# MpokiAbel/UPMEM--OpenFHE

Hardware: AMD Instinct MI355X
Metric: 64-bit coeffs/sec for NTT+Hadamard+INTT, N=2^16, 16 towers; % HBM roofline (higher is better)
Workload: dtype u64; 1 GPU; configs[2]: N=2^16, towers=16, batch=1024 per GPU, c = INTT(NTT(a) (.) b); log_n=16, towers=16, batch_per_gpu=1024, global_batch=1024, parallelism=batch-sharded x1 (no data-path collective)

## Files before the change

upmem--openfhe_amd/csrc/ntt_kernels.hpp:

```cpp
#pragma once
#include "arith.hpp"

namespace ofhe {

struct TowerConst {
    u64 q;
    u64 ninv;
    u64 ninv_pre;
    u64 mu;
    u64 nq;
    u64 nq4;
    u32 nshift;
    u32 spq_sh;
    u64 qinv;
    u32 one;
    u32 pad_;
};
#ifndef OFHE_QA_TCF
#define OFHE_QA_TCF 0
#endif
#ifndef OFHE_QA_TCI
#define OFHE_QA_TCI 0
#endif
#ifndef OFHE_QA_BLK
// ... 195 lines not shown
}
template <class M_>
__device__ __forceinline__ void dit_round16(u64 (&v)[16], const u64* dtw, u32 st, u32 r, const M_& M) {
    dit_stage16<0, 1>(v, dtw + 2 * ((u64)st + r), st, M);
    dit_stage16<1, 0>(v, dtw + 2 * ((u64)2 * st + r), st, M);
    dit_stage16<2, 1>(v, dtw + 2 * ((u64)4 * st + r), st, M);
    dit_stage16<3, 0>(v, dtw + 2 * ((u64)8 * st + r), st, M);
}

template <bool SPQ, bool QA>
__device__ __forceinline__ void dit_round3(u64 (&v)[16], const u64* dtw, const Mod<SPQ, QA>& M) {
#pragma unroll
    for (int g = 0; g < 16; g += 2) triv_bfly(v[g], v[g + 1], 2 * M.q);
#pragma unroll
    for (int g = 0; g < 16; g += 4) triv_bfly(v[g], v[g + 2], M.q4);
    {
        const Tw w = ldtw(dtw, 3);
#pragma unroll
        for (int g = 0; g < 16; g += 4) ct_bfly<0>(v[g + 1], v[g + 3], w, M);
    }
#pragma unroll
    for (int g = 0; g < 16; g += 8) triv_bfly(v[g], v[g + 4], M.q8);
#pragma unroll
    for (int j = 1; j < 4; j++) {
        const Tw w = ldtw(dtw, 4 + j);
#pragma unroll
        for (int g = 0; g < 16; g += 8) ct_bfly<0>(v[g + j], v[g + j + 4], w, M);
    }
    {
        const u64 a = red16(v[0], M), b = red16(v[8], M);
        v[0] = a;
        v[8] = b;
        triv_bfly(v[0], v[8], M.q8);
    }
#pragma unroll
    for (int j = 1; j < 8; j++) ct_bfly<1>(v[j], v[j + 8], ldtw(dtw, 8 + j), M);
}

template <bool SPQ, bool QA>
__device__ __forceinline__ u64 twist_out(u64 x, Tw f, const Mod<SPQ, QA>& M) {
    return canon4m(shoup_lazy(x, f.w, f.wp, M), M);
}

template <int S, class M_, int CS = S & 1>
__device__ __forceinline__ void fwd_stage16(u64 (&v)[16], const u64* tw, u32 M0, const M_& M) {
    constexpr int half = 8 >> S;
    const u64* base = tw + 2 * ((u64)M0 << S);
#pragma unroll
    for (int j = 0; j < (1 << S); j++) {
        Tw w = ldtw(base, j);
#pragma unroll
        for (int k = j * 2 * half; k < j * 2 * half + half; k++) ct_bfly<CS>(v[k], v[k + half], w, M);
    }
}

template <int S, class M_>
__device__ __forceinline__ void inv_stage16(u64 (&v)[16], const u64* itw, u32 M0, const M_& M) {
    constexpr int half = 8 >> S;
    const u64* base = itw + 2 * ((u64)M0 << S);
#pragma unroll
    for (int j = 0; j < (1 << S); j++) {
        Tw w = ldtw(base, j);
#pragma unroll
        for (int k = j * 2 * half; k < j * 2 * half + half; k++) gs_bfly(v[k], v[k + half], w, M);
    }
}

#ifndef OFHE_LAZY_GS
#define OFHE_LAZY_GS 1
#endif
template <class M_>
__device__ __forceinline__ void gs_bfly_b(u64& x, u64& y, Tw w, const M_& M, bool in8) {
    const u64 s = x + y;
    const u64 d = x + (in8 ? M.q8 : M.q4) - y;
    x = in8 ? red16_gs(s, M) : s;
    y = shoup_lazy(d, w.w, w.wp, M);
}
template <int S, class M_>
__device__ __forceinline__ void inv_stage16_b(u64 (&v)[16], bool (&b8)[16], const u64* itw, u32 M0, const M_& M) {
    constexpr int half = 8 >> S;
    const u64* base = itw + 2 * ((u64)M0 << S);
#pragma unroll
    for (int j = 0; j < (1 << S); j++) {
        Tw w = ldtw(base, j);
#pragma unroll
        for (int k = j * 2 * half; k < j * 2 * half + half; k++) {
            gs_bfly_b(v[k], v[k + half], w, M, b8[k] || b8[k + half]);
            b8[k] = true;
            b8[k + half] = false;
        }
    }
}
template <class M_>
__device__ __forceinline__ void inv_round16_b(u64 (&v)[16], bool (&b8)[16], const u64* itw, u32 M0, const M_& M) {
    inv_stage16_b<3>(v, b8, itw, M0, M);
    inv_stage16_b<2>(v, b8, itw, M0, M);
    inv_stage16_b<1>(v, b8, itw, M0, M);
    inv_stage16_b<0>(v, b8, itw, M0, M);
}

template <class M_>
__device__ __forceinline__ void fwd_round16(u64 (&v)[16], const u64* tw, u32 M0, const M_& M) {
    fwd_stage16<0>(v, tw, M0, M);
    fwd_stage16<1>(v, tw, M0, M);
    fwd_stage16<2>(v, tw, M0, M);
    fwd_stage16<3>(v, tw, M0, M);
}
#ifndef OFHE_FWD_CANON
#define OFHE_FWD_CANON 1
#endif
template <class M_>
__device__ __forceinline__ void fwd_round16_canon(u64 (&v)[16], const u64* tw, u32 M0, const M_& M) {
    fwd_stage16<0>(v, tw, M0, M);
    fwd_stage16<1, M_, OFHE_FWD_CANON ? 0 : 1>(v, tw, M0, M);
    fwd_stage16<2>(v, tw, M0, M);
    fwd_stage16<3>(v, tw, M0, M);
}
template <class M_>
__device__ __forceinline__ void inv_round16(u64 (&v)[16], const u64* itw, u32 M0, const M_& M) {
    inv_stage16<3>(v, itw, M0, M);
    inv_stage16<2>(v, itw, M0, M);
    inv_stage16<1>(v, itw, M0, M);
    inv_stage16<0>(v, itw, M0, M);
}

#ifndef OFHE_TW3
#define OFHE_TW3 1
#endif
#ifndef OFHE_MONT
#define OFHE_MONT 1
#endif
#ifndef OFHE_COAL
#define OFHE_COAL 1
#endif
#ifndef OFHE_COAL_B
#define OFHE_COAL_B 1
#endif
constexpr bool kMontFused = OFHE_MONT && OFHE_COAL_B;
static_assert(!(kMontFused && OFHE_THR), "Montgomery Hadamard needs the forward output < 12q");
template <int S, class M_>
__device__ __forceinline__ void fwd_stage16_t3(u64 (&v)[16], const u64* tw3, u32 U, u32 u, const M_& M) {
    constexpr int half = 8 >> S;
    const u64* base = tw3 + 2 * (u64)(((1u << S) - 1) * U);
#pragma unroll
    for (int j = 0; j < (1 << S); j++) {
        Tw w = ldtw(base + 2 * (u64)j * U, u);
#pragma unroll
        for (int k = j * 2 * half; k < j * 2 * half + half; k++) ct_bfly<S & 1>(v[k], v[k + half], w, M);
    }
}
__device__ __forceinline__ u32 lds_pad(u32 p) { return p + (p >> 4); }
constexpr u32 LDS_WORDS = 4096 + 4096 / 16;

__device__ __forceinline__ void wave_stage_in(const u64* wsrc, u64* lds, u32 tid, u64 (&out)[16]) {
    const u32 lane = tid & 63, base = (tid >> 6) * 1024;
#pragma unroll
    for (int k = 0; k < 8; k++) {
        const u64x2 v = ld2_s(wsrc + 128 * k + 2 * lane);
        const u32 p = base + 128 * k + 2 * lane;
        lds[lds_pad(p)] = v.x;
        lds[lds_pad(p) + 1] = v.y;
    }
    __builtin_amdgcn_wave_barrier();
#pragma unroll
    for (int k = 0; k < 16; k++) out[k] = lds[tid * 17 + k];
    __builtin_amdgcn_wave_barrier();
}
template <int NPRE>
__device__ __forceinline__ void wave_stage_in_pre(const u64* wsrc, u64* lds, u32 tid, const u64x2 (&pre)[NPRE > 0 ? NPRE : 1],
                                                  u64 (&out)[16]) {
    const u32 lane = tid & 63, base = (tid >> 6) * 1024;
#pragma unroll
    for (int k = 0; k < 8; k++) {
        const u64x2 v = k < NPRE ? pre[k < NPRE ? k : 0] : ld2_s(wsrc + 128 * k + 2 * lane);
        const u32 p = base + 128 * k + 2 * lane;
        lds[lds_pad(p)] = v.x;
        lds[lds_pad(p) + 1] = v.y;
    }
    __builtin_amdgcn_wave_barrier();
#pragma unroll
    for (int k = 0; k < 16; k++) out[k] = lds[tid * 17 + k];
    __builtin_amdgcn_wave_barrier();
}
__device__ __forceinline__ void wave_stage_out(const u64 (&v)[16], u64* lds, u32 tid, u64* wdst) {
    const u32 lane = tid & 63, base = (tid >> 6) * 1024;
#pragma unroll
    for (int k = 0; k < 16; k++) lds[tid * 17 + k] = v[k];
    __builtin_amdgcn_wave_barrier();
#pragma unroll
    for (int k = 0; k < 8; k++) {
        const u32 p = base + 128 * k + 2 * lane;
        u64x2 w;
        w.x = lds[lds_pad(p)];
        w.y = lds[lds_pad(p) + 1];
        st2_s(wdst + 128 * k + 2 * lane, w);
    }
}

#ifndef OFHE_B_PF
#define OFHE_B_PF 8
#endif
#ifndef OFHE_KB_WAVES
#define OFHE_KB_WAVES 4
#endif
template <int MODE, bool SPQ, int NR, int SK = 0>
__device__ __forceinline__ void block_body(const PlanArgs& P, const u64* src, u64* dst, const u64* __restrict__ bdat,
                                           u32 batch, u32 wid, u64* lds, u32 tid) {
    static_assert(NR == 2 || NR == 3, "k_block covers the last 8 (NR=2) or 12 (NR=3) stages");
    static_assert(SK == 0 || (SK == 3 && NR == 3), "k_block: SK = 3 needs NR = 3");
    const u32 logn = P.log_n;
    const u32 N = 1u << logn;
    const u32 G = N >> 12;
    const u32 g = wid % G;
    const u32 pb = wid / G;
    const u32 t = pb / batch, b = pb % batch;
    const u64 inner = (u64)t * N + ((u64)g << 12);
    const u64 off = (u64)b * P.dstride + inner;
    const u64 boff = (u64)b * P.bstride + inner;
    const u64* blk = src + (u64)b * P.sstride + inner;
    u64* oblk = dst + off;
    const TowerConst tc = P.tc[t];
    const u64 q = tc.q;
    const auto M = load_mod<SPQ, (bool)OFHE_QA_BLK>(tc);
    const u64* tw = P.tw + (u64)t * N * 2;
    const u32 h = tid >> 4, r = tid & 15;
    const u32 L1 = tid + h;
    const u32 L2 = h * 272 + r;
    const u32 L3 = tid * 17;
    u64 v[16];

    if (MODE == MODE_FWD || MODE == MODE_FUSED || MODE == MODE_FWD_SUB) {
        if (NR == 3) {
#pragma unroll
            for (int k = 0; k < 16; k++) v[k] = ld_s(blk + tid + 256 * k);
            if (SK == 3)
                fwd_stage16<3>(v, tw, (N >> 12) + g, M);
            else
                fwd_round16(v, tw, (N >> 12) + g, M);
#pragma unroll
            for (int k = 0; k < 16; k++) lds[L1 + 272 * k] = v[k];
            __syncthreads();
#pragma unroll
            for (int k = 0; k < 16; k++) v[k] = lds[L2 + 17 * k];
        } else {
#pragma unroll
            for (int k = 0; k < 16; k++) v[k] = ld_s(blk + h * 256 + r + 16 * k);
        }
        fwd_round16(v, tw, (N >> 8) + g * 16 + h, M);
#pragma unroll
        for (int k = 0; k < 16; k++) lds[L2 + 17 * k] = v[k];
        __syncthreads();
#pragma unroll
        for (int k = 0; k < 16; k++) v[k] = lds[L3 + k];
        constexpr int BPF = ((MODE == MODE_FUSED && OFHE_COAL_B) || MODE == MODE_FWD_SUB) ? OFHE_B_PF : 0;
        u64x2 bpre[BPF > 0 ? BPF : 1];
#pragma unroll
        for (int k = 0; k < BPF; k++) bpre[k] = ld2_s(bdat + boff + (tid >> 6) * 1024 + 128 * k + 2 * (tid & 63));
        if (OFHE_TW3) {
            const u64* tw3 = P.tw3 + (u64)t * (N / 16) * 30;
            const u32 U = N >> 4, u = g * 256 + tid;
            fwd_stage16_t3<0>(v, tw3, U, u, M);
            fwd_stage16_t3<1>(v, tw3, U, u, M);
            fwd_stage16_t3<2>(v, tw3, U, u, M);
            fwd_stage16_t3<3>(v, tw3, U, u, M);
        } else {
            fwd_round16(v, tw, (N >> 4) + g * 256 + tid, M);
        }
        if (!(MODE == MODE_FUSED && kMontFused) && MODE != MODE_FWD_SUB) {
#pragma unroll
            for (int k = 0; k < 16; k++) v[k] = canon_fwd<SPQ>(v[k], M);
        }
        if (MODE == MODE_FWD_SUB) {
            static_assert(!OFHE_THR, "the lazy forward-subtract needs the forward output < 12q (OFHE_THR widens it)");
            u64 xx[16];
            wave_stage_in_pre<BPF>(bdat + boff + (tid >> 6) * 1024, lds, tid, bpre, xx);
            const u64 sc = P.scal[3 * t + 1], scp = P.scal[3 * t + 2];
            const u64 q12 = M.q8 + M.q4;
#pragma unroll
            for (int k = 0; k < 16; k++) v[k] = canon4m(shoup_lazy(xx[k] + q12 - v[k], sc, scp, M), M);
            wave_stage_out(v, lds, tid, oblk + (tid >> 6) * 1024);
            return;
        }
        if (MODE == MODE_FWD) {
            if (OFHE_COAL) {
                wave_stage_out(v, lds, tid, oblk + (tid >> 6) * 1024);
            } else {
                ulonglong2* o = reinterpret_cast<ulonglong2*>(oblk + tid * 16);
#pragma unroll
                for (int k = 0; k < 8; k++) o[k] = make_ulonglong2(v[2 * k], v[2 * k + 1]);
            }
            return;
        }
        if (OFHE_COAL_B) {
            u64 bb[16];
            wave_stage_in_pre<BPF>(bdat + boff + (tid >> 6) * 1024, lds, tid, bpre, bb);
            if (kMontFused) {
#pragma unroll
                for (int k = 0; k < 16; k++) v[k] = mont_mul(v[k], bb[k], q, tc.qinv);
            } else {
#pragma unroll
                for (int k = 0; k < 16; k++) v[k] = barrett_ref(v[k], bb[k], q, tc.mu, tc.nshift);
            }
        } else {
            const ulonglong2* bp = reinterpret_cast<const ulonglong2*>(bdat + boff + tid * 16);
#pragma unroll
            for (int k = 0; k < 8; k++) {
#ifdef OFHE_ABL_NOB
                ulonglong2 bb = make_ulonglong2(v[k] ^ off, v[k + 8] ^ tid);
#else
                ulonglong2 bb = bp[k];
#endif
                v[2 * k] = barrett_ref(v[2 * k], bb.x, q, tc.mu, tc.nshift);
                v[2 * k + 1] = barrett_ref(v[2 * k + 1], bb.y, q, tc.mu, tc.nshift);
            }
        }
    } else {
        if (OFHE_COAL) {
            wave_stage_in(blk + (tid >> 6) * 1024, lds, tid, v);
        } else {
            const ulonglong2* ip = reinterpret_cast<const ulonglong2*>(blk + tid * 16);
#pragma unroll
            for (int k = 0; k < 8; k++) {
                ulonglong2 a = ip[k];
                v[2 * k] = a.x;
                v[2 * k + 1] = a.y;
            }
        }
    }
    const u64* dtw = P.dtw + (u64)t * N * 2;
    dit_round3(v, dtw, M);
#pragma unroll
    for (int k = 0; k < 16; k++) lds[L3 + k] = v[k];
    __syncthreads();
#pragma unroll
    for (int k = 0; k < 16; k++) v[k] = lds[L2 + 17 * k];
    dit_round16(v, dtw, 16, r, M);
    const u64* tw_ = P.twist + (u64)t * N * 2 + 2 * ((u64)g << 12);
    if (NR == 2) {
#pragma unroll
        for (int k = 0; k < 16; k++) {
            const u32 p = h * 256 + r + 16 * k;
            const Tw f = ldtw(tw_, p);
            st_s(oblk + p, shoup_lazy(v[k], f.w, f.wp, M));
        }
        return;
    }
#pragma unroll
    for (int k = 0; k < 16; k++) lds[L2 + 17 * k] = v[k];
    __syncthreads();
#pragma unroll
    for (int k = 0; k < 16; k++) v[k] = lds[L1 + 272 * k];
    if (SK == 3)
        dit_stage16<0, 1>(v, dtw + 2 * ((u64)256 + tid), 256, M);
    else
        dit_round16(v, dtw, 256, tid, M);
#pragma unroll
    for (int k = 0; k < 16; k++) {
        const Tw f = ldtw(tw_, tid + 256 * k);
        v[k] = logn == 12 ? twist_out(v[k], f, M) : shoup_lazy(v[k], f.w, f.wp, M);
    }
#pragma unroll
    for (int k = 0; k < 16; k++) st_s(oblk + tid + 256 * k, v[k]);
}
template <int MODE, bool SPQ, int NR, int SK = 0>
__global__ __launch_bounds__(256, OFHE_KB_WAVES) void k_block(PlanArgs P, const u64* src, u64* dst,
                                                              const u64* __restrict__ bdat, u32 batch, u32 nwg) {
    OFHE_VGPR_FLOOR();
    __shared__ u64 lds[LDS_WORDS];
    block_body<MODE, SPQ, NR, SK>(P, src, dst, bdat, batch, xcd_remap(blockIdx.x, nwg), lds, threadIdx.x);
}

struct SwSrc {
    const u64* last;
    u64 lstride;
    u64 ql;
    const u64* tab;
    u64 pre, pre_p;
};
#ifndef OFHE_TCOLS_W
#define OFHE_TCOLS_W 16
#endif
constexpr u32 TCOLS_W = OFHE_TCOLS_W;
#ifndef OFHE_TCOLS_PADF
#define OFHE_TCOLS_PADF 1
#endif
static_assert(TCOLS_W == 16 || TCOLS_W == 32, "column tile width");
constexpr u32 TCOLS_LDS_WORDS = 16 * 16 * TCOLS_W + 16 * 16;
#ifndef OFHE_TCOLS_HALF
#define OFHE_TCOLS_HALF 0
#endif
#ifndef OFHE_TCOLS_HALF_WAVES
#define OFHE_TCOLS_HALF_WAVES 5
#endif
constexpr u32 TCOLS_LDS_INV_WORDS = OFHE_TCOLS_HALF ? 8 * 16 * TCOLS_W : TCOLS_LDS_WORDS;
template <bool INV, bool SPQ, bool SWS = false, int LOGN = 16>
__device__ __forceinline__ void tcols_body(const PlanArgs& P, const u64* src, u64* dst, u32 batch, u32 wid,
                                           const SwSrc& SWA, u64* lds, u32 tid) {
    static_assert(LOGN == 16 || LOGN == 17, "k_tcols: N = 2^16 or 2^17");
    constexpr u32 N = 1u << LOGN, S = N / 256, W = TCOLS_W;
    const u32 cb = wid % (S / W);
    const u32 pb = wid / (S / W);
    const u32 t = pb / batch, b = pb % batch;
    const u64 inner = (u64)t * N + cb * W;
    const u64* x = src + (u64)b * P.sstride + inner;
    u64* y = dst + (u64)b * P.dstride + inner;
    const TowerConst tc = P.tc[t];
    const auto M = load_mod<SPQ, INV ? (bool)OFHE_QA_TCI : (bool)OFHE_QA_TCF>(tc);
    const u32 h = tid / W, r = tid % W;
    const u32 L1 = tid, L2 = h * 16 * W + r;
    u64 v[16];
    if (!INV) {
        const u64* tw = P.tw + (u64)t * N * 2;
        constexpr u32 RP = OFHE_TCOLS_PADF ? 16 * W + 16 : 16 * W;
        if (SWS) {
            const u64 w = SWA.tab[6 * t + 1], wp = SWA.tab[6 * t + 2];
            const SwMod sm = sw_mod(SWA.ql, tc.q);
            const u64* lp = SWA.last + (u64)b * SWA.lstride + cb * W;
#pragma unroll
            for (int k = 0; k < 16; k++) {
                u64 e = lp[(u64)(h + 16 * k) * S + r];
                if (SWA.pre != 1) e = shoup_canon(e, SWA.pre, SWA.pre_p, SWA.ql);
                e = switch_mod1(e, sm);
                v[k] = w != 1 ? shoup_canon(e, w, wp, tc.q) : e;
            }
        } else {
#pragma unroll
            for (int k = 0; k < 16; k++) v[k] = ld_s(x + (u64)(h + 16 * k) * S + r);
        }
        fwd_round16_canon(v, tw, 1, M);
#pragma unroll
        for (int k = 0; k < 16; k++) lds[L1 + RP * k] = v[k];
        __syncthreads();
#pragma unroll
        for (int k = 0; k < 16; k++) v[k] = lds[h * RP + r + W * k];
        fwd_round16(v, tw, 16 + h, M);
#pragma unroll
        for (int k = 0; k < 16; k++) st_s(y + (u64)(16 * h + k) * S + r, v[k]);
    } else {
        const u64* itw = P.itw + (u64)t * N * 2;
#pragma unroll
        for (int k = 0; k < 16; k++) v[k] = ld_s(x + (u64)(16 * h + k) * S + r);
        if (OFHE_LAZY_GS) {
            bool b8[16];
#pragma unroll
            for (int k = 0; k < 16; k++) b8[k] = false;
            inv_round16_b(v, b8, itw, 16 + h, M);
            if (OFHE_TCOLS_HALF) {
                u64 o[16];
                if (h < 8) {
#pragma unroll
                    for (int k = 0; k < 16; k++) lds[L2 + W * k] = v[k];
                }
                __syncthreads();
#pragma unroll
                for (int k = 0; k < 8; k++) o[k] = lds[L1 + 16 * W * k];
                __syncthreads();
                if (h >= 8) {
#pragma unroll
                    for (int k = 0; k < 16; k++) lds[L2 - 8 * 16 * W + W * k] = v[k];
                }
                __syncthreads();
#pragma unroll
                for (int k = 8; k < 16; k++) o[k] = lds[L1 + 16 * W * (k - 8)];
#pragma unroll
                for (int k = 0; k < 16; k++) {
                    v[k] = o[k];
                    b8[k] = true;
                }
            } else {
#pragma unroll
                for (int k = 0; k < 16; k++) lds[L2 + W * k] = v[k];
                __syncthreads();
#pragma unroll
                for (int k = 0; k < 16; k++) {
                    v[k] = lds[L1 + 16 * W * k];
                    b8[k] = true;
                }
            }
            inv_round16_b(v, b8, itw, 1, M);
#pragma unroll
            for (int k = 0; k < 16; k++)
                st_s(y + (u64)(h + 16 * k) * S + r, b8[k] ? canon8m(v[k], M) : canon4m(v[k], M));
        } else {
            inv_round16(v, itw, 16 + h, M);
#pragma unroll
            for (int k = 0; k < 16; k++) lds[L2 + W * k] = v[k];
            __syncthreads();
#pragma unroll
            for (int k = 0; k < 16; k++) v[k] = lds[L1 + 16 * W * k];
            inv_round16(v, itw, 1, M);
#pragma unroll
            for (int k = 0; k < 16; k++) st_s(y + (u64)(h + 16 * k) * S + r, canon4m(v[k], M));
        }
    }
}

// ... 280 lines not shown
```

upmem--openfhe_amd/csrc/ofhe_hip.hip:

```cpp
#include <cstdio>
#include <cstdlib>
#include <cstring>
#include <new>
#include <thread>

#include "compose.hpp"
#include "bconv_cols.hpp"

using namespace ofhe;

#define OFHE_VERSION "ofhe-hip 0.2 gfx950"

namespace ofhe {
static thread_local std::string g_err;
int fail(int code, const std::string& msg) {
    g_err = msg;
    return code;
}
int post_launch() {
    hipError_t e = hipGetLastError();
    if (e != hipSuccess) return fail(OFHE_ERR_HIP, std::string("kernel launch: ") + hipGetErrorString(e));
    return OFHE_OK;
}
}
// ... 346 lines not shown
    } tables[] = {{(void**)&p->d_tc, tc.data(), sizeof(TowerConst) * towers},
                  {(void**)&p->d_tw, tw.data(), words(tw)},
                  {(void**)&p->d_itw, itw.data(), words(itw)},
                  {(void**)&p->d_tw3, tw3.data(), words(tw3)},
                  {(void**)&p->d_dtw, dtw.data(), words(dtw)},
                  {(void**)&p->d_twist, twist.data(), words(twist)},
                  {(void**)&p->d_twist_r, twist_r.data(), words(twist_r)}};
    int rc = OFHE_OK;
    for (const auto& t : tables)
        if (rc == OFHE_OK) rc = alloc_upload(t.dst, t.src, t.bytes, "plan upload", ctx->device);
    if (rc != OFHE_OK) {
        ofhe_hip_plan_destroy(p);
        return rc;
    }
    *plan = p;
    return OFHE_OK;
}

int ofhe_hip_plan_tune(ofhe_plan_t p, uint32_t chunk_batch, uint32_t streams) {
    if (!p || !p->ctx) return fail(OFHE_ERR_STATE, "plan is NULL or destroyed");
    if (streams < 1 || streams > 2) return fail(OFHE_ERR_ARG, "streams must be 1 or 2");
    HIPCHK(hipSetDevice(p->ctx->device));
    std::lock_guard<std::mutex> lk(p->fork_mu);
    if (streams == 2 && !p->st[0]) {
        hipStream_t st[2] = {nullptr, nullptr};
        hipEvent_t fork = nullptr, join[2] = {nullptr, nullptr};
        hipError_t e = hipSuccess;
        for (int i = 0; i < 2 && e == hipSuccess; i++) {
            e = hipStreamCreateWithFlags(&st[i], hipStreamNonBlocking);
            if (e == hipSuccess) e = hipEventCreateWithFlags(&join[i], hipEventDisableTiming);
        }
        if (e == hipSuccess) e = hipEventCreateWithFlags(&fork, hipEventDisableTiming);
        if (e != hipSuccess) {
            for (int i = 0; i < 2; i++) {
                if (st[i]) (void)hipStreamDestroy(st[i]);
                if (join[i]) (void)hipEventDestroy(join[i]);
            }
            if (fork) (void)hipEventDestroy(fork);
            return fail(OFHE_ERR_HIP, std::string("plan_tune: ") + hipGetErrorString(e));
        }
        for (int i = 0; i < 2; i++) {
            p->st[i] = st[i];
            p->ev_join[i] = join[i];
        }
        p->ev_fork = fork;
    }
    p->chunk_batch = chunk_batch;
    p->nstreams = streams;
    return OFHE_OK;
}

int ofhe_hip_plan_destroy(ofhe_plan_t p) {
    if (!p) return fail(OFHE_ERR_ARG, "plan is NULL");
    if (p->ctx) (void)hipSetDevice(p->ctx->device);
    for (int i = 0; i < 2; i++) {
        if (p->st[i]) (void)hipStreamSynchronize(p->st[i]);
        if (p->st[i]) (void)hipStreamDestroy(p->st[i]);
        if (p->ev_join[i]) (void)hipEventDestroy(p->ev_join[i]);
    }
    if (p->ev_fork) (void)hipEventDestroy(p->ev_fork);
    (void)hipFree(p->d_tc);
    (void)hipFree(p->d_tw);
    (void)hipFree(p->d_itw);
    (void)hipFree(p->d_tw3);
    (void)hipFree(p->d_dtw);
    (void)hipFree(p->d_twist);
    (void)hipFree(p->d_twist_r);
    for (auto& kv : p->tabs) (void)hipFree(kv.second);
    delete p;
    return OFHE_OK;
}

int ofhe_hip_plan_tables(ofhe_plan_t p, uint64_t* tab, uint64_t* tab_pre, uint64_t* itab,
                         uint64_t* itab_pre, uint64_t* ninv) {
    if (!p) return fail(OFHE_ERR_ARG, "plan is NULL");
    const size_t n = p->tab.size() * sizeof(u64);
    if (tab) memcpy(tab, p->tab.data(), n);
    if (tab_pre) memcpy(tab_pre, p->tab_pre.data(), n);
    if (itab) memcpy(itab, p->itab.data(), n);
    if (itab_pre) memcpy(itab_pre, p->itab_pre.data(), n);
    if (ninv) memcpy(ninv, p->ninv.data(), p->ninv.size() * sizeof(u64));
    return OFHE_OK;
}

static PlanArgs args_of(ofhe_plan_t p, u32 t0 = 0, u32 count = 0) {
    if (!count) count = p->towers - t0;
    const u64 N = 1ull << p->log_n;
    PlanArgs a;
    a.tc = p->d_tc + t0;
    a.tw = p->d_tw + 2 * N * t0;
    a.itw = p->d_itw + 2 * N * t0;
    a.tw3 = p->d_tw3 + (N >= 4096 ? (N / 16) * 30 * t0 : 0);
    a.sstride = a.dstride = a.bstride = N * count;
    a.scal = nullptr;
    a.dtw = p->d_dtw + 2 * N * t0;
    a.twist = p->d_twist + 2 * N * t0;
    a.log_n = p->log_n;
    a.towers = count;
    return a;
}

static PlanArgs fused_args(ofhe_plan_t p) {
    PlanArgs a = args_of(p);
    if (kMontFused && p->log_n >= 12) a.twist = p->d_twist_r;
    return a;
}

static int check_common(ofhe_plan_t p, uint32_t batch) {
    if (!p || !p->ctx) return fail(OFHE_ERR_STATE, "plan is NULL or destroyed");
    if (batch == 0) return fail(OFHE_ERR_ARG, "batch must be >= 1");
    const u64 polys = (u64)batch * p->towers;
    if (polys * ((u64)1 << p->log_n) / 4096 >= (1ull << 31))
        return fail(OFHE_ERR_ARG, "batch too large for one launch");
    return OFHE_OK;
}

#ifndef OFHE_COLS_CPT
#define OFHE_COLS_CPT 2
#endif
static void launch_colpass(const PlanArgs& a, bool spq, int split, bool inv, const u64* src, u64* dst, u32 batch,
                           hipStream_t s, const SwSrc* lift = nullptr) {
    const SwSrc S = lift ? *lift : SwSrc{nullptr, 0, 0, nullptr, 1, 0};
    const u32 polys = batch * a.towers;
    with_bool(spq, [&](auto sp) { with_bool(inv, [&](auto iv) { with_bool(lift != nullptr, [&](auto sw) {
        constexpr bool SP = decltype(sp)::value, INV = decltype(iv)::value, SWS = decltype(sw)::value;
        if constexpr (!(INV && SWS)) {
            if (split == SPLIT_T9) {
                if constexpr (!SWS) {
                    const u32 nwg = polys * 16;
                    hipLaunchKernelGGL((k_tcols9<INV, SP>), dim3(nwg), dim3(512), 0, s, a, src, dst, batch, nwg);
                }
            } else if (split != SPLIT_COLS) {
                with_int<16, 17>(split == SPLIT_T8B9 ? 17 : 16, [&](auto ln) {
                    constexpr int LOGN = decltype(ln)::value;
                    const u32 nwg = polys * ((1u << (LOGN - 8)) / TCOLS_W);
                    hipLaunchKernelGGL((k_tcols<INV, SP, SWS, LOGN>), dim3(nwg), dim3(16 * TCOLS_W), 0, s, a, src,
                                       dst, batch, nwg, S);
                });
            } else {
                with_int<1, 2, 3, 4, 5>((int)a.log_n - 12, [&](auto ka) {
                    constexpr int KA = decltype(ka)::value, CPT = KA <= 4 ? OFHE_COLS_CPT : 1;
                    const u32 nwg = polys * (16 / CPT);
                    hipLaunchKernelGGL((k_cols<KA, INV, CPT, SP, SWS>), dim3(nwg), dim3(256), 0, s, a, src, dst,
                                       batch, nwg, S);
                });
            }
        }
    }); }); });
}

template <int MODE>
static void launch_block(const PlanArgs& a, bool spq, const u64* src, u64* dst, const u64* b, u32 batch,
                         hipStream_t s, int split = SPLIT_COLS) {
    const u32 nwg = batch * a.towers * (1u << (a.log_n - 12));
    with_bool(spq, [&](auto sp) { with_int<8, 9, 12>((int)block_stages(split, a.log_n), [&](auto st) {
        constexpr int NR = decltype(st)::value == 8 ? 2 : 3, SK = decltype(st)::value == 9 ? 3 : 0;
        hipLaunchKernelGGL((k_block<MODE, decltype(sp)::value, NR, SK>), dim3(nwg), dim3(256), 0, s, a, src, dst, b,
                           batch, nwg);
    }); });
}

template <int MODE>
static void launch_small(const PlanArgs& a, bool spq, const u64* src, u64* dst, const u64* b, u32 batch,
                         hipStream_t s) {
    const u32 N = 1u << a.log_n;
    const u32 thr = N / 2 >= 256 ? 256 : (N / 2 < 64 ? 64 : N / 2);
    with_bool(spq, [&](auto sp) {
        hipLaunchKernelGGL((k_small<MODE, decltype(sp)::value>), dim3(batch * a.towers), dim3(thr), 0, s, a, src, dst,
                           b, batch);
    });
}


namespace ofhe {
int plan_ntt_range(ofhe_plan_t p, bool inverse, u32 t0, u32 count, const u64* src, u64* dst, u64 sstride,
                   u64 dstride, u32 batch, hipStream_t s) {
    if (!p || !p->ctx) return fail(OFHE_ERR_STATE, "plan is NULL or destroyed");
    if (count == 0 || batch == 0) return OFHE_OK;
    if (t0 + count > p->towers || t0 + count < t0) return fail(OFHE_ERR_ARG, "tower range outside the plan");
    if (!src || !dst) return fail(OFHE_ERR_ARG, "data is NULL");
    const u64 N = 1ull << p->log_n;
    if (sstride < N * count || dstride < N * count)
        return fail(OFHE_ERR_ARG, "batch stride smaller than the tower range");
    if ((u64)batch * count * N / 4096 >= (1ull << 31)) return fail(OFHE_ERR_ARG, "batch too large for one launch");
    HIPCHK(hipSetDevice(p->ctx->device));
    PlanArgs a = args_of(p, t0, count);
    PlanArgs ad = a;
    a.sstride = sstride;
    a.dstride = ad.sstride = ad.dstride = dstride;
    if (!inverse) {
        if (p->log_n < 12) {
            launch_small<MODE_FWD>(a, p->spq, src, dst, nullptr, batch, s);
        } else if (p->log_n == 12) {
            launch_block<MODE_FWD>(a, p->spq, src, dst, nullptr, batch, s, p->split);
        } else {
            launch_colpass(a, p->spq, p->split, false, src, dst, batch, s);
            launch_block<MODE_FWD>(ad, p->spq, dst, dst, nullptr, batch, s, p->split);
        }
    } else {
        if (p->log_n < 12) {
            launch_small<MODE_INV>(a, p->spq, src, dst, nullptr, batch, s);
        } else {
            launch_block<MODE_INV>(a, p->spq, src, dst, nullptr, batch, s, p->split);
            if (p->log_n > 12) launch_colpass(ad, p->spq, p->split, true, dst, dst, batch, s);
        }
    }
    return post_launch();
}

int plan_cols_switch(ofhe_plan_t p, u32 t0, u32 count, const u64* last, u64 lstride, u64 ql, u64 pre, const u64* tab,
                     u64* y, u64 ystride, u32 batch, hipStream_t s) {
    if (!p || !p->ctx) return fail(OFHE_ERR_STATE, "plan is NULL or destroyed");
    if (p->log_n <= 12 || p->split == SPLIT_T9) return fail(OFHE_ERR_ARG, "plan_cols_switch: k_cols / k_tcols plans only");
    if (((uintptr_t)last & 15) || (lstride & 1)) return fail(OFHE_ERR_ARG, "plan_cols_switch: misaligned source");
    HIPCHK(hipSetDevice(p->ctx->device));
    PlanArgs a = args_of(p, t0, count);
    a.sstride = a.dstride = ystride;
    pre %= ql;
    const SwSrc S{last, lstride, ql, tab, pre, pre == 1 ? 0 : shoup_pre(pre, ql)};
    launch_colpass(a, p->spq, p->split, false, nullptr, y, batch, s, &S);
    return post_launch();
}

int plan_ntt_fwd_block(ofhe_plan_t p, u32 t0, u32 count, u64* y, u64 ystride, u32 batch, hipStream_t s) {
    if (!p || !p->ctx) return fail(OFHE_ERR_STATE, "plan is NULL or destroyed");
    if (p->log_n <= 12) return fail(OFHE_ERR_ARG, "plan_ntt_fwd_block: log_n > 12 only");
    HIPCHK(hipSetDevice(p->ctx->device));
    PlanArgs a = args_of(p, t0, count);
    a.sstride = a.dstride = ystride;
    launch_block<MODE_FWD>(a, p->spq, y, y, nullptr, batch, s, p->split);
    return post_launch();
}

int plan_ntt_inv_block(ofhe_plan_t p, u32 t0, u32 count, const u64* src, u64 sstride, u64* dst, u64 dstride, u32 batch,
                       hipStream_t s) {
    if (!p || !p->ctx) return fail(OFHE_ERR_STATE, "plan is NULL or destroyed");
    if (p->log_n <= 12) return fail(OFHE_ERR_ARG, "plan_ntt_inv_block: log_n > 12 only");
    if (count == 0 || batch == 0) return OFHE_OK;
    if (t0 + count > p->towers) return fail(OFHE_ERR_ARG, "tower range outside the plan");
    HIPCHK(hipSetDevice(p->ctx->device));
    PlanArgs a = args_of(p, t0, count);
    a.sstride = sstride;
    a.dstride = dstride;
    launch_block<MODE_INV>(a, p->spq, src, dst, nullptr, batch, s, p->split);
    return post_launch();
}

int plan_ntt_fwd_sub(ofhe_plan_t p, u32 t0, u32 count, u64* y, u64 ystride, const u64* x, u64 xstride, u64* out,
                     u64 ostride, const u64* scal, u32 batch, hipStream_t s, int parts) {
    if (!p || !p->ctx) return fail(OFHE_ERR_STATE, "plan is NULL or destroyed");
    if (p->log_n < 12) return fail(OFHE_ERR_ARG, "fused forward + subtract needs log_n >= 12");
    if (count == 0 || batch == 0) return OFHE_OK;
    if (t0 + count > p->towers) return fail(OFHE_ERR_ARG, "tower range outside the plan");
    HIPCHK(hipSetDevice(p->ctx->device));
    PlanArgs a = args_of(p, t0, count);
    a.sstride = a.dstride = ystride;
    if (p->log_n > 12 && (parts & 1)) launch_colpass(a, p->spq, p->split, false, y, y, batch, s);
    if (!(parts & 2)) return post_launch();
    PlanArgs ab = a;
    ab.sstride = ystride;
    ab.dstride = ostride;
    ab.bstride = xstride;
    ab.scal = scal;
    launch_block<MODE_FWD_SUB>(ab, p->spq, y, out, x, batch, s, p->split);
    return post_launch();
}
}

int ofhe_hip_ntt_fwd(ofhe_plan_t p, uint64_t* data, uint32_t batch, void* stream) {
    RCCHK(check_common(p, batch));
    if (!data) return fail(OFHE_ERR_ARG, "data is NULL");
    const u64 d = (u64)p->towers << p->log_n;
    return plan_ntt_range(p, false, 0, p->towers, data, data, d, d, batch, pick(stream));
}

int ofhe_hip_ntt_inv(ofhe_plan_t p, uint64_t* data, uint32_t batch, void* stream) {
    RCCHK(check_common(p, batch));
    if (!data) return fail(OFHE_ERR_ARG, "data is NULL");
    const u64 d = (u64)p->towers << p->log_n;
    return plan_ntt_range(p, true, 0, p->towers, data, data, d, d, batch, pick(stream));
}

int ofhe_hip_ntt_fwd_range(ofhe_plan_t p, uint32_t t0, uint32_t count, const uint64_t* src, uint64_t* dst,
                           uint64_t src_stride, uint64_t dst_stride, uint32_t batch, void* stream) {
    if (!p || !p->ctx) return fail(OFHE_ERR_STATE, "plan is NULL or destroyed");
    if (batch == 0 || count == 0) return fail(OFHE_ERR_ARG, "batch and count must be >= 1");
    return plan_ntt_range(p, false, t0, count, src, dst, src_stride, dst_stride, batch, pick(stream));
}

int ofhe_hip_ntt_inv_range(ofhe_plan_t p, uint32_t t0, uint32_t count, const uint64_t* src, uint64_t* dst,
                           uint64_t src_stride, uint64_t dst_stride, uint32_t batch, void* stream) {
    if (!p || !p->ctx) return fail(OFHE_ERR_STATE, "plan is NULL or destroyed");
    if (batch == 0 || count == 0) return fail(OFHE_ERR_ARG, "batch and count must be >= 1");
    return plan_ntt_range(p, true, t0, count, src, dst, src_stride, dst_stride, batch, pick(stream));
}

int ofhe_hip_ntt_mul_intt(ofhe_plan_t p, const uint64_t* a_, const uint64_t* b, uint64_t* c,
                          uint32_t batch, void* stream) {
    int rc = check_common(p, batch);
    if (rc) return rc;
    if (!a_ || !b || !c) return fail(OFHE_ERR_ARG, "NULL data pointer");
    if (b == c && a_ != c) return fail(OFHE_ERR_ARG, "c may alias a but not b");
    HIPCHK(hipSetDevice(p->ctx->device));
    const PlanArgs a = fused_args(p);
    hipStream_t s = pick(stream);
    if (p->log_n < 12) {
        launch_small<MODE_FUSED>(a, p->spq, a_, c, b, batch, s);
    } else if (p->log_n == 12) {
        launch_block<MODE_FUSED>(a, p->spq, a_, c, b, batch, s, p->split);
// ... 451 lines not shown
```

Before: 77.66 billion coeffs/s.

## Remap NR=2 block kernel to 16-thread teams with wave-local sync

For the 8-stage block path, each 16-thread team now owns a separate 256-coefficient chunk. Each wave covers four batch entries at one chunk position, so the workgroup-wide __syncthreads between stages becomes a wave barrier. The grid is resized to match, and a live mask guards the padded batch tail. This removes block-level barrier stalls and lets waves progress independently, at the cost of scattered global access across batch entries and redundant work for padded lanes.

```diff
diff --git a/upmem--openfhe_amd/csrc/ntt_kernels.hpp b/upmem--openfhe_amd/csrc/ntt_kernels.hpp
--- a/upmem--openfhe_amd/csrc/ntt_kernels.hpp
+++ b/upmem--openfhe_amd/csrc/ntt_kernels.hpp
@@ -371,48 +371,59 @@
 __device__ __forceinline__ u32 lds_pad(u32 p) { return p + (p >> 4); }
 constexpr u32 LDS_WORDS = 4096 + 4096 / 16;
 
+template <bool TEAM>
+struct StageMap {
+    u32 l, base;
+    static constexpr u32 E = TEAM ? 32 : 128;
+    __device__ __forceinline__ explicit StageMap(u32 tid)
+        : l(TEAM ? (tid & 15) : (tid & 63)), base(TEAM ? (tid >> 4) * 256 : (tid >> 6) * 1024) {}
+    __device__ __forceinline__ u32 g(int k) const { return E * k + 2 * l; }
+    __device__ __forceinline__ u32 p(int k) const { return lds_pad(base + g(k)); }
+};
+template <bool TEAM>
 __device__ __forceinline__ void wave_stage_in(const u64* wsrc, u64* lds, u32 tid, u64 (&out)[16]) {
-    const u32 lane = tid & 63, base = (tid >> 6) * 1024;
+    const StageMap<TEAM> m(tid);
 #pragma unroll
     for (int k = 0; k < 8; k++) {
-        const u64x2 v = ld2_s(wsrc + 128 * k + 2 * lane);
-        const u32 p = base + 128 * k + 2 * lane;
-        lds[lds_pad(p)] = v.x;
-        lds[lds_pad(p) + 1] = v.y;
+        const u64x2 v = ld2_s(wsrc + m.g(k));
+        lds[m.p(k)] = v.x;
+        lds[m.p(k) + 1] = v.y;
     }
     __builtin_amdgcn_wave_barrier();
 #pragma unroll
     for (int k = 0; k < 16; k++) out[k] = lds[tid * 17 + k];
     __builtin_amdgcn_wave_barrier();
 }
-template <int NPRE>
+template <bool TEAM, int NPRE>
 __device__ __forceinline__ void wave_stage_in_pre(const u64* wsrc, u64* lds, u32 tid, const u64x2 (&pre)[NPRE > 0 ? NPRE : 1],
                                                   u64 (&out)[16]) {
-    const u32 lane = tid & 63, base = (tid >> 6) * 1024;
+    const StageMap<TEAM> m(tid);
 #pragma unroll
     for (int k = 0; k < 8; k++) {
-        const u64x2 v = k < NPRE ? pre[k < NPRE ? k : 0] : ld2_s(wsrc + 128 * k + 2 * lane);
-        const u32 p = base + 128 * k + 2 * lane;
-        lds[lds_pad(p)] = v.x;
-        lds[lds_pad(p) + 1] = v.y;
+        const u64x2 v = k < NPRE ? pre[k < NPRE ? k : 0] : ld2_s(wsrc + m.g(k));
+        lds[m.p(k)] = v.x;
+        lds[m.p(k) + 1] = v.y;
     }
     __builtin_amdgcn_wave_barrier();
 #pragma unroll
     for (int k = 0; k < 16; k++) out[k] = lds[tid * 17 + k];
     __builtin_amdgcn_wave_barrier();
 }
-__device__ __forceinline__ void wave_stage_out(const u64 (&v)[16], u64* lds, u32 tid, u64* wdst) {
-    const u32 lane = tid & 63, base = (tid >> 6) * 1024;
+template <bool TEAM>
+__device__ __forceinline__ void wave_stage_out(const u64 (&v)[16], u64* lds, u32 tid, u64* wdst, bool live = true) {
+    const StageMap<TEAM> m(tid);
 #pragma unroll
     for (int k = 0; k < 16; k++) lds[tid * 17 + k] = v[k];
     __builtin_amdgcn_wave_barrier();
+    u64x2 w[8];
 #pragma unroll
     for (int k = 0; k < 8; k++) {
-        const u32 p = base + 128 * k + 2 * lane;
-        u64x2 w;
-        w.x = lds[lds_pad(p)];
-        w.y = lds[lds_pad(p) + 1];
-        st2_s(wdst + 128 * k + 2 * lane, w);
+        w[k].x = lds[m.p(k)];
+        w[k].y = lds[m.p(k) + 1];
+    }
+    if (live) {
+#pragma unroll
+        for (int k = 0; k < 8; k++) st2_s(wdst + m.g(k), w[k]);
     }
 }
 
@@ -422,27 +433,51 @@
 #ifndef OFHE_KB_WAVES
 #define OFHE_KB_WAVES 4
 #endif
+template <int NR>
+__device__ __forceinline__ void block_sync() {
+    if (NR == 2)
+        __builtin_amdgcn_wave_barrier();
+    else
+        __syncthreads();
+}
 template <int MODE, bool SPQ, int NR, int SK = 0>
 __device__ __forceinline__ void block_body(const PlanArgs& P, const u64* src, u64* dst, const u64* __restrict__ bdat,
                                            u32 batch, u32 wid, u64* lds, u32 tid) {
     static_assert(NR == 2 || NR == 3, "k_block covers the last 8 (NR=2) or 12 (NR=3) stages");
     static_assert(SK == 0 || (SK == 3 && NR == 3), "k_block: SK = 3 needs NR = 3");
+    constexpr bool TEAM = NR == 2;
     const u32 logn = P.log_n;
     const u32 N = 1u << logn;
-    const u32 G = N >> 12;
-    const u32 g = wid % G;
-    const u32 pb = wid / G;
-    const u32 t = pb / batch, b = pb % batch;
-    const u64 inner = (u64)t * N + ((u64)g << 12);
+    const u32 h = tid >> 4, r = tid & 15;
+    u32 g, t, b;
+    bool live = true;
+    if (TEAM) {
+        const u32 G4 = N >> 10, nq = (batch + 3) >> 2;
+        const u32 wave = __builtin_amdgcn_readfirstlane(tid >> 6);
+        g = (wid % G4) * 4 + wave;
+        const u32 pq = wid / G4;
+        t = pq / nq;
+        const u32 bt = (pq % nq) * 4 + (h & 3);
+        live = bt < batch;
+        b = live ? bt : batch - 1;
+    } else {
+        const u32 G = N >> 12;
+        g = wid % G;
+        const u32 pb = wid / G;
+        t = pb / batch;
+        b = pb % batch;
+    }
+    const u64 inner = (u64)t * N + ((u64)g << (TEAM ? 8 : 12));
     const u64 off = (u64)b * P.dstride + inner;
     const u64 boff = (u64)b * P.bstride + inner;
+    const u32 wq = TEAM ? 0 : (tid >> 6) * 1024;
     const u64* blk = src + (u64)b * P.sstride + inner;
     u64* oblk = dst + off;
+    const u32 e3 = (TEAM ? r : tid) * 16;
     const TowerConst tc = P.tc[t];
     const u64 q = tc.q;
     const auto M = load_mod<SPQ, (bool)OFHE_QA_BLK>(tc);
     const u64* tw = P.tw + (u64)t * N * 2;
-    const u32 h = tid >> 4, r = tid & 15;
     const u32 L1 = tid + h;
     const u32 L2 = h * 272 + r;
     const u32 L3 = tid * 17;
@@ -463,27 +498,27 @@
             for (int k = 0; k < 16; k++) v[k] = lds[L2 + 17 * k];
         } else {
 #pragma unroll
-            for (int k = 0; k < 16; k++) v[k] = ld_s(blk + h * 256 + r + 16 * k);
-        }
-        fwd_round16(v, tw, (N >> 8) + g * 16 + h, M);
+            for (int k = 0; k < 16; k++) v[k] = ld_s(blk + r + 16 * k);
+        }
+        fwd_round16(v, tw, (N >> 8) + (TEAM ? g : g * 16 + h), M);
 #pragma unroll
         for (int k = 0; k < 16; k++) lds[L2 + 17 * k] = v[k];
-        __syncthreads();
+        block_sync<NR>();
 #pragma unroll
         for (int k = 0; k < 16; k++) v[k] = lds[L3 + k];
         constexpr int BPF = ((MODE == MODE_FUSED && OFHE_COAL_B) || MODE == MODE_FWD_SUB) ? OFHE_B_PF : 0;
         u64x2 bpre[BPF > 0 ? BPF : 1];
 #pragma unroll
-        for (int k = 0; k < BPF; k++) bpre[k] = ld2_s(bdat + boff + (tid >> 6) * 1024 + 128 * k + 2 * (tid & 63));
+        for (int k = 0; k < BPF; k++) bpre[k] = ld2_s(bdat + boff + wq + StageMap<TEAM>(tid).g(k));
         if (OFHE_TW3) {
             const u64* tw3 = P.tw3 + (u64)t * (N / 16) * 30;
-            const u32 U = N >> 4, u = g * 256 + tid;
+            const u32 U = N >> 4, u = TEAM ? g * 16 + r : g * 256 + tid;
             fwd_stage16_t3<0>(v, tw3, U, u, M);
             fwd_stage16_t3<1>(v, tw3, U, u, M);
             fwd_stage16_t3<2>(v, tw3, U, u, M);
             fwd_stage16_t3<3>(v, tw3, U, u, M);
         } else {
-            fwd_round16(v, tw, (N >> 4) + g * 256 + tid, M);
+            fwd_round16(v, tw, (N >> 4) + (TEAM ? g * 16 + r : g * 256 + tid), M);
         }
         if (!(MODE == MODE_FUSED && kMontFused) && MODE != MODE_FWD_SUB) {
 #pragma unroll
@@ -492,27 +527,27 @@
         if (MODE == MODE_FWD_SUB) {
             static_assert(!OFHE_THR, "the lazy forward-subtract needs the forward output < 12q (OFHE_THR widens it)");
             u64 xx[16];
-            wave_stage_in_pre<BPF>(bdat + boff + (tid >> 6) * 1024, lds, tid, bpre, xx);
+            wave_stage_in_pre<TEAM, BPF>(bdat + boff + wq, lds, tid, bpre, xx);
             const u64 sc = P.scal[3 * t + 1], scp = P.scal[3 * t + 2];
             const u64 q12 = M.q8 + M.q4;
 #pragma unroll
             for (int k = 0; k < 16; k++) v[k] = canon4m(shoup_lazy(xx[k] + q12 - v[k], sc, scp, M), M);
-            wave_stage_out(v, lds, tid, oblk + (tid >> 6) * 1024);
+            wave_stage_out<TEAM>(v, lds, tid, oblk + wq, live);
             return;
         }
         if (MODE == MODE_FWD) {
             if (OFHE_COAL) {
-                wave_stage_out(v, lds, tid, oblk + (tid >> 6) * 1024);
+                wave_stage_out<TEAM>(v, lds, tid, oblk + wq, live);
             } else {
-                ulonglong2* o = reinterpret_cast<ulonglong2*>(oblk + tid * 16);
-#pragma unroll
-                for (int k = 0; k < 8; k++) o[k] = make_ulonglong2(v[2 * k], v[2 * k + 1]);
+                ulonglong2* o = reinterpret_cast<ulonglong2*>(oblk + e3);
+#pragma unroll
+                for (int k = 0; k < 8 && live; k++) o[k] = make_ulonglong2(v[2 * k], v[2 * k + 1]);
             }
             return;
         }
         if (OFHE_COAL_B) {
             u64 bb[16];
-            wave_stage_in_pre<BPF>(bdat + boff + (tid >> 6) * 1024, lds, tid, bpre, bb);
+            wave_stage_in_pre<TEAM, BPF>(bdat + boff + wq, lds, tid, bpre, bb);
             if (kMontFused) {
 #pragma unroll
                 for (int k = 0; k < 16; k++) v[k] = mont_mul(v[k], bb[k], q, tc.qinv);
@@ -521,7 +556,7 @@
                 for (int k = 0; k < 16; k++) v[k] = barrett_ref(v[k], bb[k], q, tc.mu, tc.nshift);
             }
         } else {
-            const ulonglong2* bp = reinterpret_cast<const ulonglong2*>(bdat + boff + tid * 16);
+            const ulonglong2* bp = reinterpret_cast<const ulonglong2*>(bdat + boff + e3);
 #pragma unroll
             for (int k = 0; k < 8; k++) {
 #ifdef OFHE_ABL_NOB
@@ -535,9 +570,9 @@
         }
     } else {
         if (OFHE_COAL) {
-            wave_stage_in(blk + (tid >> 6) * 1024, lds, tid, v);
+            wave_stage_in<TEAM>(blk + wq, lds, tid, v);
         } else {
-            const ulonglong2* ip = reinterpret_cast<const ulonglong2*>(blk + tid * 16);
+            const ulonglong2* ip = reinterpret_cast<const ulonglong2*>(blk + e3);
 #pragma unroll
             for (int k = 0; k < 8; k++) {
                 ulonglong2 a = ip[k];
@@ -550,17 +585,20 @@
     dit_round3(v, dtw, M);
 #pragma unroll
     for (int k = 0; k < 16; k++) lds[L3 + k] = v[k];
-    __syncthreads();
+    block_sync<NR>();
 #pragma unroll
     for (int k = 0; k < 16; k++) v[k] = lds[L2 + 17 * k];
     dit_round16(v, dtw, 16, r, M);
-    const u64* tw_ = P.twist + (u64)t * N * 2 + 2 * ((u64)g << 12);
+    const u64* tw_ = P.twist + (u64)t * N * 2 + 2 * ((u64)g << (TEAM ? 8 : 12));
     if (NR == 2) {
 #pragma unroll
         for (int k = 0; k < 16; k++) {
-            const u32 p = h * 256 + r + 16 * k;
-            const Tw f = ldtw(tw_, p);
-            st_s(oblk + p, shoup_lazy(v[k], f.w, f.wp, M));
+            const Tw f = ldtw(tw_, r + 16 * k);
+            v[k] = shoup_lazy(v[k], f.w, f.wp, M);
+        }
+        if (live) {
+#pragma unroll
+            for (int k = 0; k < 16; k++) st_s(oblk + r + 16 * k, v[k]);
         }
         return;
     }
diff --git a/upmem--openfhe_amd/csrc/ofhe_hip.hip b/upmem--openfhe_amd/csrc/ofhe_hip.hip
--- a/upmem--openfhe_amd/csrc/ofhe_hip.hip
+++ b/upmem--openfhe_amd/csrc/ofhe_hip.hip
@@ -522,9 +522,10 @@
 template <int MODE>
 static void launch_block(const PlanArgs& a, bool spq, const u64* src, u64* dst, const u64* b, u32 batch,
                          hipStream_t s, int split = SPLIT_COLS) {
-    const u32 nwg = batch * a.towers * (1u << (a.log_n - 12));
     with_bool(spq, [&](auto sp) { with_int<8, 9, 12>((int)block_stages(split, a.log_n), [&](auto st) {
         constexpr int NR = decltype(st)::value == 8 ? 2 : 3, SK = decltype(st)::value == 9 ? 3 : 0;
+        const u32 nwg = NR == 2 ? ((batch + 3) / 4) * a.towers * (1u << (a.log_n - 10))
+                                : batch * a.towers * (1u << (a.log_n - 12));
         hipLaunchKernelGGL((k_block<MODE, decltype(sp)::value, NR, SK>), dim3(nwg), dim3(256), 0, s, a, src, dst, b,
                            batch, nwg);
     }); });
```

Measured after the change: 79.72 billion coeffs/s (median of 6 runs). 1.03x the previous value.
